# SpeakerGuard/SpeakerGuard

Hardware: AMD Instinct MI355X
Metric: PGD attack steps/sec (xv_plda, 3s@16kHz, batch 64) (higher is better)
Workload: dtype f32; 1 GPU; PGD L-inf eps=0.002 step=0.0004 CE untargeted on xv_plda CSI-E, 64 x 3 s @ 16 kHz per GPU (every rank its own batch), EOT 1/1, dither off; timed = K steps + final forward-only pass; median of 5 attacks; batch_per_gpu=64, samples=48000, global_batch=64

## Files before the change

### speakerguard_amd/csrc/k_conv_gemm.hip

```cpp
#include <atomic>
#include <cstdio>
#include <cstdlib>
#include <vector>
#include <type_traits>

#include "sg_internal.h"

namespace sg {

typedef float f32x16 __attribute__((ext_vector_type(16)));
typedef int i32x4 __attribute__((ext_vector_type(4)));
typedef float f32x4 __attribute__((ext_vector_type(4)));

constexpr int BK = 32;

template <int BM, int BN, int WM, int WN>
__device__ __forceinline__ void gemm_segment(const ConvGemmArgs& p, float* smem, int m0, int n0, int c_begin,
                                             int c_end, f32x16 (&acc)[BM / WM / 32][BN / WN / 32]) {
    constexpr int MI = BM / WM / 32;
    constexpr int NI = BN / WN / 32;
    constexpr int A_QUADS = BM / 4;
    constexpr int B_F4 = BK * BN / 4;
    constexpr int B_PER_THREAD = (B_F4 + 255) / 256;
    static_assert(A_QUADS * 8 <= 256, "A tile too tall");
// ... 708 lines not shown
#pragma unroll
                for (int mi = 0; mi < MI; ++mi) {
                    const float4 x = oa[cur][mi][g];
                    const float xa = st == 0 ? x.x : st == 1 ? x.y : st == 2 ? x.z : x.w;
#pragma unroll
                    for (int ni = 0; ni < NI; ++ni) {
                        const float4 y = BG ? obr[J % DB][ni][h * KGS + g] : ob[cur][ni][g];
                        const float yb = st == 0 ? y.x : st == 1 ? y.y : st == 2 ? y.z : y.w;
                        acc[mi][ni] = __builtin_amdgcn_mfma_f32_32x32x2f32(xa, yb, acc[mi][ni], 0, 0, 0);
                    }
                }
            }
        }
        __builtin_amdgcn_sched_barrier(0);
        __syncthreads();
    };
    const int trips = n / 6;
    for (int q = 0; q < trips; ++q) {
        chunk(std::integral_constant<int, 0>{});
        chunk(std::integral_constant<int, 1>{});
        chunk(std::integral_constant<int, 2>{});
        chunk(std::integral_constant<int, 3>{});
        chunk(std::integral_constant<int, 4>{});
        chunk(std::integral_constant<int, 5>{});
    }
    const int rest = n - 6 * trips;
    if (rest >= 1) chunk(std::integral_constant<int, 0>{});
    if (rest >= 2) chunk(std::integral_constant<int, 1>{});
    if (rest >= 3) chunk(std::integral_constant<int, 2>{});
    if (rest >= 4) chunk(std::integral_constant<int, 3>{});
    if (rest >= 5) chunk(std::integral_constant<int, 4>{});
}

template <int BM, int BN, int WM, int WN, int EPI>
__device__ __forceinline__ void tile_store(const ConvGemmArgs& p, float* C, int m0, int n0,
                                           f32x16 (&acc)[BM / WM / 32][BN / WN / 32]) {
    constexpr int MI = BM / WM / 32;
    constexpr int NI = BN / WN / 32;
    const int lane = threadIdx.x & 63;
    const int wid = __builtin_amdgcn_readfirstlane(threadIdx.x >> 6);
    const int wm = wid / WN, wn = wid % WN;
    const int l31 = lane & 31, lhi = lane >> 5;
    const unsigned lane_off = (unsigned)(4 * lhi * p.ldc + l31) * 4u;
#pragma unroll
    for (int mi = 0; mi < MI; ++mi) {
        const int rowu = m0 + wm * (BM / WM) + mi * 32;
        if (rowu + 32 <= p.M) {
#pragma unroll
            for (int ni = 0; ni < NI; ++ni) {
                const int colu = n0 + wn * (BN / WN) + ni * 32;
                const size_t base = (size_t)rowu * p.ldc + colu;
                float bias = 0.f;
                if (EPI == EPI_BIAS_RELU) bias = p.bias[colu + l31];
                f32x16 mk;
                if (EPI == EPI_RELU_MASK) {
#pragma unroll
                    for (int e = 0; e < 16; ++e) {
                        const char* mb = reinterpret_cast<const char*>(p.mask + base + (size_t)((e & 3) + 8 * (e >> 2)) * p.ldc);
                        mk[e] = *reinterpret_cast<const float*>(mb + lane_off);
                    }
                }
#pragma unroll
                for (int e = 0; e < 16; ++e) {
                    float v = acc[mi][ni][e];
                    if (EPI == EPI_BIAS_RELU) v = fmaxf(v + bias, 0.f);
                    if (EPI == EPI_RELU_MASK) v = mk[e] > 0.f ? v : 0.f;
                    char* cb = reinterpret_cast<char*>(C + base + (size_t)((e & 3) + 8 * (e >> 2)) * p.ldc);
                    *reinterpret_cast<float*>(cb + lane_off) = v;
                }
            }
        } else if (rowu < p.M) {
#pragma unroll
            for (int ni = 0; ni < NI; ++ni) {
                const int col = n0 + wn * (BN / WN) + ni * 32 + l31;
                const int row0 = rowu + 4 * lhi;
                float bias = 0.f;
                if (EPI == EPI_BIAS_RELU) bias = p.bias[col];
                f32x16 mk;
                if (EPI == EPI_RELU_MASK) {
#pragma unroll
                    for (int e = 0; e < 16; ++e) {
                        const int row = min(row0 + (e & 3) + 8 * (e >> 2), p.M - 1);
                        mk[e] = p.mask[(size_t)row * p.ldc + col];
                    }
                }
#pragma unroll
                for (int e = 0; e < 16; ++e) {
                    const int row = row0 + (e & 3) + 8 * (e >> 2);
                    float v = acc[mi][ni][e];
                    if (EPI == EPI_BIAS_RELU) v = fmaxf(v + bias, 0.f);
                    if (EPI == EPI_RELU_MASK) v = mk[e] > 0.f ? v : 0.f;
                    if (row < p.M) C[(size_t)row * p.ldc + col] = v;
                }
            }
        }
    }
}

template <int MI, int NI>
__device__ __forceinline__ void acc_zero(f32x16 (&acc)[MI][NI]) {
#pragma unroll
    for (int mi = 0; mi < MI; ++mi)
#pragma unroll
        for (int ni = 0; ni < NI; ++ni)
#pragma unroll
            for (int e = 0; e < 16; ++e) acc[mi][ni][e] = 0.f;
}

template <int BM, int BN, int WM, int WN, int EPI>
__global__ __launch_bounds__(256, 2) void conv_gemm_kernel(ConvGemmArgs p, int mtiles, int ntiles) {
    __shared__ __attribute__((aligned(16))) float smem[2 * BK * (BM + BN)];
    const int nblk = mtiles * ntiles;
    int bid = blockIdx.x;
    {
        const int q = nblk / 8, r = nblk % 8;
        const int xcd = bid % 8, loc = bid / 8;
        bid = (xcd < r ? xcd * (q + 1) : r * (q + 1) + (xcd - r) * q) + loc;
    }
    const int mt = bid / ntiles, nt = bid % ntiles;
    const int m0 = mt * BM, n0 = nt * BN;
    const int c_begin = blockIdx.z * p.chunks_per_split;
    const int c_end = min(p.total_chunks, c_begin + p.chunks_per_split);
    f32x16 acc[BM / WM / 32][BN / WN / 32];
    acc_zero(acc);
    gemm_segment<BM, BN, WM, WN>(p, smem, m0, n0, c_begin, c_end, acc);
// ... 164 lines not shown
            while (__hip_atomic_load(flags + w - 1, __ATOMIC_RELAXED, __HIP_MEMORY_SCOPE_AGENT) != epoch) {
                __builtin_amdgcn_s_sleep(8);
                if (++spins > ((p.ablate & 8) ? (1u << 12) : (1u << 26))) {
                    if (p.err_word) __hip_atomic_fetch_or(p.err_word, 1u, __ATOMIC_RELAXED, __HIP_MEMORY_SCOPE_SYSTEM);
                    break;
                }
            }
        }
        if (p.ablate & 16) __builtin_amdgcn_fence(__ATOMIC_ACQUIRE, "agent");
        __syncthreads();
        SG_STAMP(9)
        if (computing) {
#pragma unroll
            for (int mi = 0; mi < MI; ++mi)
#pragma unroll
                for (int ni = 0; ni < NI; ++ni)
#pragma unroll
                    for (int q = 0; q < 4; ++q) {
                        const f32x4 v = __builtin_bit_cast(f32x4, __builtin_amdgcn_raw_buffer_load_b128(slab_rsrc, piece_off(w - 1, mi, ni, q), 0, 16));
                        acc[mi][ni][4 * q] = v.x; acc[mi][ni][4 * q + 1] = v.y; acc[mi][ni][4 * q + 2] = v.z; acc[mi][ni][4 * q + 3] = v.w;
                    }
        }
        const int c1 = first_tile == last_tile ? last_c1 : C;
        SG_STAMP(10)
        segment(m0, n0, first_c0, c1, p.trace ? p.trace + (size_t)w * 16 : nullptr);
        SG_STAMP(11)
        if (computing) tile_store<BM, BN, WM, WN, EPI>(p, p.C, m0, n0, acc);
        SG_STAMP(12)
    }
    if (sk_deep(KIND) && p.trace && threadIdx.x == 0) p.trace[(size_t)w * 16 + 14] = __builtin_readcyclecounter();
#undef SG_STAMP
}

template <int BM, int BN, int WM, int WN>
static hipError_t launch_tile(const ConvGemmArgs& a, int epi, int splits, hipStream_t s) {
    const int mtiles = (a.M + BM - 1) / BM;
    const int ntiles = a.N / BN;
    dim3 grid(mtiles * ntiles, 1, splits);
    switch (epi) {
        case EPI_NONE:
            hipLaunchKernelGGL((conv_gemm_kernel<BM, BN, WM, WN, EPI_NONE>), grid, dim3(256), 0, s, a, mtiles, ntiles);
            break;
        case EPI_BIAS_RELU:
            hipLaunchKernelGGL((conv_gemm_kernel<BM, BN, WM, WN, EPI_BIAS_RELU>), grid, dim3(256), 0, s, a, mtiles, ntiles);
            break;
        case EPI_RELU_MASK:
            hipLaunchKernelGGL((conv_gemm_kernel<BM, BN, WM, WN, EPI_RELU_MASK>), grid, dim3(256), 0, s, a, mtiles, ntiles);
            break;
        default:
            return hipErrorInvalidValue;
    }
    return hipGetLastError();
}

typedef float f32x4 __attribute__((ext_vector_type(4)));
template <int EPI, int D, bool TRACE>
__global__ __launch_bounds__(256) void conv_gemm_s16_kernel(ConvGemmArgs p, int ntile32) {
    static_assert(D % 3 == 0, "the LDS stage of a chunk is taken from its ring slot");
    constexpr int A_STAGE = 32 * 32, STAGE = A_STAGE + 8 * 32 * 4;
    __shared__ __attribute__((aligned(16))) float smem[3 * STAGE];
    const int tid = threadIdx.x, lane = tid & 63, wid = tid >> 6;
    const int bm0 = ((int)blockIdx.x / ntile32) * 32, bn0 = ((int)blockIdx.x % ntile32) * 32;
    constexpr unsigned kOob = 0x80000000u;
    const int srow = bm0 + (tid >> 3), c4 = tid & 7;
    const bool srow_ok = srow < p.M;
    const int sb = srow_ok ? srow / p.Tc : 0;
// ... 165 lines not shown
template <int EPI, int KIND>
static void launch_streamk_kind(const ConvGemmArgs& a, int workers, int ntiles, int tiles, int ipw, float* slabs,
                                unsigned* flags, unsigned epoch, hipStream_t s) {
    constexpr int threads = sk_threads(KIND);
    constexpr size_t lds = sk_lds_bytes(KIND);
    static std::atomic<unsigned long long> done_mask{0};
    int dev = 0;
    (void)hipGetDevice(&dev);
    const unsigned long long bit = 1ull << (dev & 63);
    if (!(done_mask.load(std::memory_order_relaxed) & bit)) {
        (void)hipFuncSetAttribute(reinterpret_cast<const void*>(conv_gemm_streamk_kernel<EPI, KIND>),
                                  hipFuncAttributeMaxDynamicSharedMemorySize, (int)lds);
        done_mask.fetch_or(bit, std::memory_order_relaxed);
    }
    hipLaunchKernelGGL((conv_gemm_streamk_kernel<EPI, KIND>), dim3(workers), dim3(threads), lds, s, a, ntiles,
                       tiles, ipw, slabs, flags, epoch);
}

template <int KIND>
static int streamk_blocks_per_cu() {
    static const int n = [] {
        constexpr size_t lds = sk_lds_bytes(KIND);
        const void* fn = reinterpret_cast<const void*>(conv_gemm_streamk_kernel<EPI_NONE, KIND>);
        (void)hipFuncSetAttribute(fn, hipFuncAttributeMaxDynamicSharedMemorySize, (int)lds);
        int nb = 0;
        if (hipOccupancyMaxActiveBlocksPerMultiprocessor(&nb, conv_gemm_streamk_kernel<EPI_NONE, KIND>, sk_threads(KIND), lds) !=
            hipSuccess)
            nb = 0;
        return nb;
    }();
    return n;
}

static hipError_t launch_streamk(const ConvGemmArgs& a, int epi, float* slabs, unsigned* flags, hipStream_t s) {
    static const int w16 = [] {
        const char* e = sg_tune_env("SG_STREAMK_W16");
        return e ? atoi(e) : 1;
    }();
    int kind = !a.Wq ? 0 : ((w16 && a.force != 3) ? 2 : 1);
    const int cus = a.num_cus > 0 && a.num_cus < 256 ? a.num_cus : 256;
    int bm = kind == 2 ? 256 : 128, workers = kind == 2 ? cus : 2 * cus;
    static const int mid = [] {
        const char* e = sg_tune_env("SG_STREAMK_MID");
        return e ? atoi(e) : 1;
    }();
    static const int mid9 = [] {
        const char* e = sg_tune_env("SG_STREAMK_MID9");
        return e ? atoi(e) : 0;
    }();
    if (mid && kind == 2 && a.force == 0 && ((a.M + 255) / 256) * (a.N / 128) < cus) {
        static const int deep = [] {
            const char* e = sg_tune_env("SG_STREAMK_DEEP");
            return e ? atoi(e) : 1;
        }();
        if (((a.M + 127) / 128) * (a.N / 128) >= cus) {
            kind = deep ? (mid9 ? 9 : 5) : 1;
            bm = 128;
            workers = cus;
        } else if (((a.M + 63) / 64) * (a.N / 128) >= cus) {
            kind = deep ? 6 : 3;
            bm = 64;
            workers = cus;
        } else if (((a.M + 31) / 32) * (a.N / 128) >= cus) {
            kind = deep ? 7 : 4;
            bm = 32;
            workers = cus;
        }
// ... 7 lines not shown
        return e ? atoi(e) : 64;
    }();

    if (ws256 && kind == 2 && a.force == 0) {
        if (a.total_chunks >= ws256_min_chunks) {
            kind = 8;
        } else {
            kind = 5;
            bm = 128;
            workers = cus;
        }
    }
    static const int env_kind = [] {
        const char* e = sg_tune_env("SG_STREAMK_KIND");
        return e ? atoi(e) : 0;
    }();
    if (env_kind >= 5 && env_kind <= 9 && a.force == 0 && a.Wq) {
        const int kind0 = kind, bm0 = bm, workers0 = workers;
        kind = env_kind;
        bm = kind == 5 || kind == 9 ? 128 : kind == 6 ? 64 : kind == 7 ? 32 : 256;
        workers = cus;
        const long tl = (long)((a.M + bm - 1) / bm) * (a.N / 128);
        if (tl < workers || (tl * a.total_chunks + workers - 1) / workers < a.total_chunks) {
            kind = kind0;
            bm = bm0;
            workers = workers0;
        }
    }
    if (a.force >= 6 && a.force <= 10 && a.Wq) {
        kind = a.force - 1;
        bm = kind == 5 || kind == 9 ? 128 : kind == 6 ? 64 : kind == 7 ? 32 : 256;
        workers = cus;
    }
    const int mtiles = (a.M + bm - 1) / bm, ntiles = a.N / 128;
    const int tiles = mtiles * ntiles;
    const long total = (long)tiles * a.total_chunks;
    const int ipw = (int)((total + workers - 1) / workers);
    static const int min_chunks = [] {
        const char* e = sg_tune_env("SG_STREAMK_MINCHUNKS");
        return e ? atoi(e) : 16;
    }();
    if (!slabs || !flags || tiles < workers || ipw < a.total_chunks || a.total_chunks < min_chunks) return hipErrorNotSupported;
    const int per_cu = kind == 2 ? streamk_blocks_per_cu<2>() : kind == 1 ? streamk_blocks_per_cu<1>()
                     : kind == 3 ? streamk_blocks_per_cu<3>() : kind == 4 ? streamk_blocks_per_cu<4>()
                     : kind == 5 ? streamk_blocks_per_cu<5>() : kind == 6 ? streamk_blocks_per_cu<6>()
                     : kind == 7 ? streamk_blocks_per_cu<7>() : kind == 8 ? streamk_blocks_per_cu<8>() : kind == 9 ? streamk_blocks_per_cu<9>() : streamk_blocks_per_cu<0>();
    if ((long)per_cu * cus < workers) return hipErrorNotSupported;
    if ((size_t)workers * bm * 128 > (size_t)512 * 128 * 128) return hipErrorNotSupported;
    static std::atomic<unsigned> launch_counter{0};
    unsigned epoch = ++launch_counter;
    if (epoch == 0) epoch = ++launch_counter;
    static const char* trace_file = sg_tune_env("SG_SK_TRACE");
    static const long trace_skip = [] {
        const char* e = sg_tune_env("SG_SK_TRACE_SKIP");
        return e ? atol(e) : 0L;
    }();
    static const long trace_count = [] {
        const char* e = sg_tune_env("SG_SK_TRACE_COUNT");
        return e ? atol(e) : (1L << 60);
    }();
    static std::atomic<long> trace_seen{0};
    static PerDeviceScratch trace_buf;
    bool trace_this = trace_file != nullptr;
    if (trace_this) {
        const long idx = trace_seen.fetch_add(1, std::memory_order_relaxed);
        trace_this = idx >= trace_skip && idx - trace_skip < trace_count;
    }
    unsigned long long* trace_dev = trace_this ? static_cast<unsigned long long*>(trace_buf.get((size_t)workers * 16 * 8)) : nullptr;
    ConvGemmArgs at = a;
    at.trace = trace_dev;
    if (at.lose_counter && *at.lose_counter > 0) {
        at.ablate |= 8;
        --*at.lose_counter;
    }
    at.lose_counter = nullptr;
    dim3 grid(workers);
#define a at
#define SG_SK(EPI)                                                                                          \
    if (kind == 9) launch_streamk_kind<EPI, 9>(a, workers, ntiles, tiles, ipw, slabs, flags, epoch, s);       \
    else if (kind == 8) launch_streamk_kind<EPI, 8>(a, workers, ntiles, tiles, ipw, slabs, flags, epoch, s);  \
    else if (kind == 7) launch_streamk_kind<EPI, 7>(a, workers, ntiles, tiles, ipw, slabs, flags, epoch, s);  \
    else if (kind == 6) launch_streamk_kind<EPI, 6>(a, workers, ntiles, tiles, ipw, slabs, flags, epoch, s);  \
    else if (kind == 5) launch_streamk_kind<EPI, 5>(a, workers, ntiles, tiles, ipw, slabs, flags, epoch, s);  \
    else if (kind == 4) launch_streamk_kind<EPI, 4>(a, workers, ntiles, tiles, ipw, slabs, flags, epoch, s);  \
    else if (kind == 3) launch_streamk_kind<EPI, 3>(a, workers, ntiles, tiles, ipw, slabs, flags, epoch, s);  \
    else if (kind == 2) launch_streamk_kind<EPI, 2>(a, workers, ntiles, tiles, ipw, slabs, flags, epoch, s);  \
    else if (kind == 1) launch_streamk_kind<EPI, 1>(a, workers, ntiles, tiles, ipw, slabs, flags, epoch, s);  \
    else launch_streamk_kind<EPI, 0>(a, workers, ntiles, tiles, ipw, slabs, flags, epoch, s);
    switch (epi) {
        case EPI_NONE: SG_SK(EPI_NONE) break;
        case EPI_BIAS_RELU: SG_SK(EPI_BIAS_RELU) break;
        case EPI_RELU_MASK: SG_SK(EPI_RELU_MASK) break;
        default: return hipErrorInvalidValue;
    }
#undef SG_SK
#undef a
    if (trace_this && trace_dev) {
        std::vector<unsigned long long> h((size_t)workers * 16);
        if (hipStreamSynchronize(s) == hipSuccess &&
            hipMemcpy(h.data(), trace_dev, h.size() * 8, hipMemcpyDeviceToHost) == hipSuccess) {
            if (FILE* f = fopen(trace_file, "ab")) {
                const int hdr[8] = {workers, at.M, at.N, at.total_chunks, ipw, tiles, epi, 0};
                fwrite(hdr, sizeof(hdr), 1, f);
                fwrite(h.data(), 8, h.size(), f);
                fclose(f);
            }
        }
    }
    return hipGetLastError();
}

__global__ void pack_k4_kernel(const float* __restrict__ w, int K, int N, float* __restrict__ wq) {
    const size_t i = (size_t)blockIdx.x * blockDim.x + threadIdx.x;
    if (i >= (size_t)K * N) return;
    const int k = (int)(i / N), n = (int)(i % N);
    wq[((size_t)(k >> 2) * N + n) * 4 + (k & 3)] = w[i];
}

hipError_t launch_pack_k4(const float* w, int K, int N, float* wq, hipStream_t s) {
    const size_t n = (size_t)K * N;
    hipLaunchKernelGGL(pack_k4_kernel, dim3((unsigned)((n + 255) / 256)), dim3(256), 0, s, w, K, N, wq);
    return hipGetLastError();
}

int conv_gemm_tile_rows(int M, int N) {
    (void)M;
    (void)N;
    return 64;
}

hipError_t launch_conv_gemm(const ConvGemmArgs& a_in, int tile, int epi, int splits, hipStream_t s) {
#ifdef SG_EXP_ABLATE
    static const int ablate = [] {
        const char* e = sg_tune_env("SG_ABLATE");
        return e ? atoi(e) : 0;
    }();
#else
    constexpr int ablate = 0;
#endif
    static const int use_streamk = [] {
        const char* e = sg_tune_env("SG_STREAMK");
        return e ? atoi(e) : 1;
    }();
    ConvGemmArgs a = a_in;
    a.ablate |= ablate;
    static const int sk_xcd = [] {
        const char* e = sg_tune_env("SG_STREAMK_XCD");
        return e ? atoi(e) : 2;
    }();
    a.sk_xcd = sk_xcd;
    static const int use_quad = [] {
        const char* e = sg_tune_env("SG_QUADFEED");
        return e ? atoi(e) : 1;
    }();
    if (!use_quad || a.force == 2 || (a.ldw % 4) || (a.Kc % 4)) a.Wq = nullptr;
    if (a.Kc % BK != 0 || a.M <= 0 || a.Tc <= 0) return hipErrorInvalidValue;
    const size_t a_bytes = (size_t)(a.M / a.Tc) * a.Ta * a.lda * sizeof(float);
    const size_t w_bytes = (size_t)a.taps * a.Kc * a.ldw * sizeof(float);
    if (a_bytes >= 0x80000000ull || w_bytes >= 0x80000000ull) return hipErrorInvalidValue;
    a.a_bytes = (unsigned)a_bytes;
    a.w_bytes = (unsigned)w_bytes;
    static const long s16_max = [] {
        const char* e = sg_tune_env("SG_S16_MAX_BLOCKS");
        return e ? atol(e) : 2800L;
    }();
    if ((tile == 0 || tile == 2) && splits == 1 && a.Wq && (a.N % 32) == 0 &&
        (a.force == 5 || (a.force == 0 && a.total_chunks >= 4 && (long)((a.M + 15) / 16) * (a.N / 16) <= s16_max)))
        return launch_s16(a, epi, s);
    switch (tile) {
        case 0: {
            if (a.N % 128) return hipErrorInvalidValue;
            if (splits == 1 && use_streamk && !a.no_streamk && a.force != 1 && a.force != 4) {
                const hipError_t e = launch_streamk(a, epi, a.sk_slabs, a.sk_flags, s);
                if (e != hipErrorNotSupported) return e;
                if (a.force >= 6) return hipErrorInvalidValue;
            }
            if (a.Wq && splits == 1 && a.force != 1) return launch_tile_q(a, epi, s);
            return launch_tile<64, 128, 2, 2>(a, epi, splits, s);
        }
        case 1:
            if (a.N % 32) return hipErrorInvalidValue;
            return launch_tile<128, 32, 4, 1>(a, epi, splits, s);
        case 2:
            if (a.N % 128) return hipErrorInvalidValue;
            if (a.Wq && splits == 1 && a.force != 1) return launch_tile_q(a, epi, s);
            return launch_tile<64, 128, 2, 2>(a, epi, splits, s);
        default:
            return hipErrorInvalidValue;
    }
}

}
```

### speakerguard_amd/csrc/sg_api.hip

```cpp
#include <algorithm>
#include <cmath>
#include <cstdarg>
#include <cstdio>
#include <cstdlib>
#include <cstring>
#include <memory>
#include <type_traits>

#include "sg_internal.h"

using namespace sg;

namespace {

int fail(sg_ctx* ctx, int code, const char* fmt, ...) {
    char buf[512];
    va_list ap;
    va_start(ap, fmt);
    vsnprintf(buf, sizeof(buf), fmt, ap);
    va_end(ap);
    if (ctx) ctx->err = buf;
    return code;
}

// ... 248 lines not shown
    return SG_OK;
}

ConvGemmArgs fwd_layer_args(sg_ctx* ctx, int l, int B, int F) {
    const Workspace& w = ctx->ws;
    ConvGemmArgs a{};
    a.A = l == 0 ? w.feats : w.act[l - 1];
    a.W = ctx->xv.wf[l];
    a.Wq = ctx->xv.wfq[l];
    a.C = w.act[l];
    a.bias = ctx->xv.bias[l];
    a.mask = nullptr;
    a.Ta = l == 0 ? F : w.Fl[l - 1];
    a.Tc = w.Fl[l];
    a.M = B * a.Tc;
    a.N = kCoutPad[l];
    a.Kc = kCinPad[l];
    a.lda = kCinPad[l];
    a.ldw = kCoutPad[l];
    a.ldc = kCoutPad[l];
    a.taps = kTaps[l];
    a.tap_step = kDil[l];
    a.total_chunks = a.taps * (a.Kc / 32);
    a.chunks_per_split = a.total_chunks;
    a.split_stride = 0;
    conv_ctx_args(ctx, a);
    return a;
}

int run_tdnn_forward(sg_ctx* ctx, const PassDims& d, hipStream_t s) {
    Workspace& w = ctx->ws;
    for (int l = 0; l < kLayers; ++l) {
        ConvGemmArgs a = fwd_layer_args(ctx, l, d.B, d.F);
        SG_STAGE(l + 1, launch_conv_gemm(a, 0, EPI_BIAS_RELU, 1, s));
    }
    SG_STAGE(SG_STAGE_POOL_FWD, launch_pool_fwd(w.act[4], d.B, w.Fl[4], w.stats, s));
    ConvGemmArgs a{};
    a.A = w.stats; a.W = ctx->xv.fc1_w; a.C = w.fc1_part; a.bias = nullptr; a.mask = nullptr;
    a.M = d.B; a.N = kEmb; a.Ta = 1; a.Tc = 1; a.Kc = kStats; a.lda = kStats; a.ldw = kEmb; a.ldc = kEmb;
    a.taps = 1; a.tap_step = 0; a.total_chunks = kStats / 32;
    a.chunks_per_split = a.total_chunks / kFc1SplitK;
    a.split_stride = (long long)d.B * kEmb;
    SG_STAGE(SG_STAGE_FC1_FWD, launch_conv_gemm(a, 2, EPI_NONE, kFc1SplitK, s));
    return SG_OK;
}

int run_tdnn_backward(sg_ctx* ctx, const PassDims& d, hipStream_t s) {
    Workspace& w = ctx->ws;
    {
        ConvGemmArgs a{};
        a.A = w.demb; a.W = ctx->xv.fc1_wt; a.C = w.dstats_part; a.bias = nullptr; a.mask = nullptr;
        a.M = d.B; a.N = kStats; a.Ta = 1; a.Tc = 1; a.Kc = kEmb; a.lda = kEmb; a.ldw = kStats; a.ldc = kStats;
        a.taps = 1; a.tap_step = 0; a.total_chunks = kEmb / 32;
        a.chunks_per_split = a.total_chunks / kFc1BwdSplitK;
        a.split_stride = (long long)d.B * kStats;
        SG_STAGE(SG_STAGE_FC1_BWD, launch_conv_gemm(a, 2, EPI_NONE, kFc1BwdSplitK, s));
    }
    SG_STAGE(SG_STAGE_POOL_BWD, launch_pool_bwd(w.act[4], w.stats, w.dstats_part, kFc1BwdSplitK, d.B, w.Fl[4], w.dact[4], s));
    for (int l = kLayers - 1; l >= 0; --l) {
        ConvGemmArgs a{};
        a.A = w.dact[l];
        a.W = ctx->xv.wb[l];
        a.Wq = ctx->xv.wbq[l];
            a.C = l == 0 ? w.dfeats : w.dact[l - 1];
        a.bias = nullptr;
        a.mask = l == 0 ? nullptr : w.act[l - 1];
        a.Ta = w.Fl[l];
        a.Tc = l == 0 ? d.F : w.Fl[l - 1];
        a.M = d.B * a.Tc;
        a.N = kCinPad[l];
        a.Kc = kCoutPad[l];
        a.lda = kCoutPad[l];
        a.ldw = kCinPad[l];
        a.ldc = kCinPad[l];
        a.taps = kTaps[l];
        a.tap_step = -kDil[l];
        a.total_chunks = a.taps * (a.Kc / 32);
        a.chunks_per_split = a.total_chunks;
        a.split_stride = 0;
        conv_ctx_args(ctx, a);
        int splits = 1, tile = 0;
        if (l == 0) {
            tile = 1;
            splits = kL1BwdSplitK;
            a.chunks_per_split = a.total_chunks / kL1BwdSplitK;
            a.split_stride = (long long)d.B * d.F * kFeatPad;
        }
        SG_STAGE(-(l + 1), launch_conv_gemm(a, tile, l == 0 ? EPI_NONE : EPI_RELU_MASK, splits, s));
    }
    return SG_OK;
}

int check_dims(sg_ctx* ctx, int B, int TF, int flag, PassDims* d) {
    if (!ctx) return SG_ERR_ARG;
    if (!ctx->xv.loaded) return fail(ctx, SG_ERR_STATE, "no x-vector model loaded (call sg_xv_load)");
    if (int h = sg_health(ctx)) return h;
    SG_HIP(hipSetDevice(ctx->device));
    if (B < 1) return fail(ctx, SG_ERR_ARG, "B must be >= 1");
    if (flag < 0 || flag > 2) return fail(ctx, SG_ERR_ARG, "flag must be 0 (wav), 1 (raw feat) or 2 (cmvn feat)");
    d->B = B;
    if (flag == SG_FLAG_WAV) {
        if (TF < kWin) return fail(ctx, SG_ERR_ARG, "waveform shorter than one 25 ms window");
        d->T = TF;
        d->F = num_frames(TF);
    } else {
        d->T = 0;
        d->F = TF;
    }
    int Fl[kLayers];
    if (!layer_frames(d->F, Fl)) return fail(ctx, SG_ERR_ARG, "%d frames are too few for the TDNN context", d->F);
    {
        size_t worst = 0;
        for (int l = 0; l < kLayers; ++l) {
// ... 664 lines not shown
```

### speakerguard_amd/csrc/sg_internal.h

```cpp
#pragma once
#include <hip/hip_runtime.h>
#include <cstdlib>
#include <stdint.h>
#include <string>
#include <vector>

#include "../../include/speakerguard_hip.h"

namespace sg {

constexpr int kShift = 160;
constexpr int kWin = 400;
constexpr int kFft = 512;
constexpr int kMel = 30;
constexpr int kCep = 30;
constexpr int kLdaLd = 516;
constexpr int kFeatPad = 32;
constexpr int kCmnWindow = 300;
constexpr float kEps = 1.1920928955078125e-07f;

constexpr int kLayers = 5;
constexpr int kCin[kLayers] = {30, 512, 512, 512, 512};
constexpr int kCout[kLayers] = {512, 512, 512, 512, 1500};
constexpr int kCinPad[kLayers] = {32, 512, 512, 512, 512};
// ... 287 lines not shown
constexpr int kMaxDevices = 64;
inline int sg_device_slot() {
    int d = 0;
    (void)hipGetDevice(&d);
    return d & (kMaxDevices - 1);
}
struct PerDeviceScratch {
    void* ptr[kMaxDevices] = {};
    size_t cap[kMaxDevices] = {};
    void* get(size_t bytes) {
        const int d = sg_device_slot();
        if (cap[d] < bytes) {
            if (ptr[d]) (void)hipFree(ptr[d]);
            ptr[d] = nullptr;
            cap[d] = 0;
            if (hipMalloc(&ptr[d], bytes) == hipSuccess) cap[d] = bytes;
        }
        return ptr[d];
    }
};

inline void conv_ctx_args(sg_ctx* ctx, ConvGemmArgs& a) {
    a.sk_slabs = ctx->sk_slabs;
    a.sk_flags = ctx->sk_flags;
    a.err_word = ctx->err_dev;
    a.num_cus = ctx->num_cus;
    a.no_streamk = ctx->use_streamk ? 0 : 1;
    a.ablate = 0;
    a.lose_counter = ctx->use_streamk ? &ctx->lose_handoffs : nullptr;
}

hipError_t launch_conv_gemm(const ConvGemmArgs& a, int tile, int epi, int splits, hipStream_t s);
int conv_gemm_tile_rows(int M, int N);
hipError_t launch_pack_k4(const float* w, int K, int N, float* wq, hipStream_t s);

hipError_t launch_input_scale(const float* x, int64_t n, float* scratch512, float* scale, int mode, hipStream_t s);
hipError_t launch_mfcc_fwd(const MfccTables& t, const float* x, int B, int T, int F, const float* scale,
                           const sg_dither* dz, float* feats, hipStream_t s);
hipError_t launch_mfcc_bwd(const MfccTables& t, const float* x, int B, int T, int F, const float* scale,
                           const sg_dither* dz, const float* dfeats, float* dframes, hipStream_t s);
hipError_t launch_frames_to_wave(const float* dframes, int B, int T, int F, int R, const float* acc_in, float* grad_out,
                                 float* x_io, const float* lower, const float* upper, float step, int grad_sign,
                                 hipStream_t s);
hipError_t launch_pgd_update(float* x, const float* g, const float* lo, const float* hi, int64_t n,
                             float step, int grad_sign, hipStream_t s);
hipError_t launch_copy_cols(const float* in, int ld_in, float* out, int ld_out, int64_t rows, int ncol, hipStream_t s);
hipError_t launch_sum_cols(const float* in, int ld_in, int nsplit, long long slab_stride, float* out, int ld_out,
                           int64_t rows, int ncol, hipStream_t s);
hipError_t launch_cmvn_fwd(const float* in, int ld_in, float* out, int ld_out, int B, int F, hipStream_t s);
hipError_t launch_cmvn_bwd(const float* dout, int ld_dout, int nsplit, long long slab_stride, float* din, int ld_din,
                           int B, int F, hipStream_t s);
hipError_t launch_pool_fwd(const float* act5, int B, int Tc, float* stats, hipStream_t s);
hipError_t launch_pool_bwd(const float* act5, const float* stats, const float* dstats_part, int nsplit,
                           int B, int Tc, float* dact5, hipStream_t s);

hipError_t launch_cw2_step(float* modifier, float* exp_avg, float* exp_avg_sq, const float* x, const float* input_cur,
                           const float* grad1, const float* const_c, int B, int T, float lr, int step_t,
                           float* input_next, float* loss2, float* scratch, hipStream_t s);
hipError_t launch_nes_queries(const float* x, int n, int T, int half, int with_clean, float sigma, uint64_t seed,
                              int64_t index_base, int pair_base, const float* noise_in, float* queries, float* noise_out,
                              hipStream_t s);
hipError_t launch_nes_grad(const float* loss, int n, int T, int half, int with_clean, uint64_t seed, int64_t index_base,
                           int pair_base, const float* noise_in, int accumulate, float final_sigma, int final_batches,
                           float* grad, hipStream_t s);
hipError_t launch_fakebob_step(float* x, float* grad, const float* prev_grad, const float* lr, const float* lower,
                               const float* upper, int n, int T, float momentum, float one_m_momentum, int grad_sign,
// ... 71 lines not shown
```

Before: 407.2 steps/s.

## Chain two consecutive 1x1 conv GEMMs into one persistent stream-K launch

Adds a chained stream-K kernel that runs two back-to-back 1x1 layer GEMMs (forward layers 4-5 and backward dgrad layers 5-4) inside a single persistent launch. Each worker publishes per-worker completion flags after the first GEMM, and the second GEMM's staging waves spin only on the flags covering the row-tiles they need, so the second layer can start before the whole first layer finishes. The intent is to remove a kernel boundary and its tail/drain idle time. The cost is first-layer stores done as agent-scope atomic writes, extra spin-waits, and more complex host planning that falls back when the chain is not supported.

```diff
diff --git a/speakerguard_amd/csrc/k_conv_gemm.hip b/speakerguard_amd/csrc/k_conv_gemm.hip
--- a/speakerguard_amd/csrc/k_conv_gemm.hip
+++ b/speakerguard_amd/csrc/k_conv_gemm.hip
@@ -764,7 +764,7 @@
     if (rest >= 5) chunk(std::integral_constant<int, 4>{});
 }
 
-template <int BM, int BN, int WM, int WN, int EPI>
+template <int BM, int BN, int WM, int WN, int EPI, bool WT = false>
 __device__ __forceinline__ void tile_store(const ConvGemmArgs& p, float* C, int m0, int n0,
                                            f32x16 (&acc)[BM / WM / 32][BN / WN / 32]) {
     constexpr int MI = BM / WM / 32;
@@ -798,7 +798,8 @@
                     if (EPI == EPI_BIAS_RELU) v = fmaxf(v + bias, 0.f);
                     if (EPI == EPI_RELU_MASK) v = mk[e] > 0.f ? v : 0.f;
                     char* cb = reinterpret_cast<char*>(C + base + (size_t)((e & 3) + 8 * (e >> 2)) * p.ldc);
-                    *reinterpret_cast<float*>(cb + lane_off) = v;
+                    if constexpr (WT) __hip_atomic_store(reinterpret_cast<float*>(cb + lane_off), v, __ATOMIC_RELAXED, __HIP_MEMORY_SCOPE_AGENT);
+                    else *reinterpret_cast<float*>(cb + lane_off) = v;
                 }
             }
         } else if (rowu < p.M) {
@@ -822,7 +823,10 @@
                     float v = acc[mi][ni][e];
                     if (EPI == EPI_BIAS_RELU) v = fmaxf(v + bias, 0.f);
                     if (EPI == EPI_RELU_MASK) v = mk[e] > 0.f ? v : 0.f;
-                    if (row < p.M) C[(size_t)row * p.ldc + col] = v;
+                    if (row < p.M) {
+                        if constexpr (WT) __hip_atomic_store(C + (size_t)row * p.ldc + col, v, __ATOMIC_RELAXED, __HIP_MEMORY_SCOPE_AGENT);
+                        else C[(size_t)row * p.ldc + col] = v;
+                    }
                 }
             }
         }
@@ -1053,6 +1057,153 @@
 #undef SG_STAMP
 }
 
+constexpr int kChainFlagStride = 256;
+template <int EPI, int KIND>
+__global__ __launch_bounds__(sk_threads(KIND), sk_min_waves(KIND)) void conv_gemm_chain_kernel(ConvGemmArgs p1, ConvGemmArgs p2, int mtiles,
+                                                                                    int ntiles1, int ntiles2, int ipw1, int ipw2,
+                                                                                    float* slabs, unsigned* flags, unsigned epoch) {
+    static_assert(KIND >= 5 && KIND <= 7, "the chained launch runs the wave-specialised 128- / 64- / 32-row kinds");
+    constexpr int WM = sk_wm(KIND), WN = sk_wn(KIND);
+    constexpr int BM = sk_bm(KIND), BN = 128;
+    constexpr int MI = BM / WM / 32, NI = BN / WN / 32;
+    constexpr bool BG = sk_bg(KIND);
+    extern __shared__ __attribute__((aligned(16))) float smem[];
+    const int per_xcd = gridDim.x >> 3;
+    const int w = (p1.sk_xcd && (gridDim.x & 7) == 0) ? (blockIdx.x & 7) * per_xcd + (blockIdx.x >> 3) : blockIdx.x;
+    const int lane = threadIdx.x & 63, wid = threadIdx.x >> 6;
+    const bool staging = __builtin_amdgcn_readfirstlane(wid) >= WM * WN;
+    unsigned* const done = flags + 2 * kChainFlagStride;
+    unsigned long long* const tr = p1.trace ? p1.trace + (size_t)w * 16 : nullptr;
+    if (tr && threadIdx.x == 0) {
+        unsigned hw, xcc;
+        asm volatile("s_getreg_b32 %0, hwreg(HW_REG_HW_ID)" : "=s"(hw));
+        asm volatile("s_getreg_b32 %0, hwreg(HW_REG_XCC_ID)" : "=s"(xcc));
+        tr[15] = ((unsigned long long)xcc << 32) | hw;
+        for (int i = 1; i < 15; ++i) tr[i] = 0;
+        tr[0] = __builtin_amdgcn_s_memrealtime();
+    }
+    const unsigned spin_cap = (p1.ablate & 8) ? (1u << 12) : (1u << 26);
+    auto give_up = [&]() {
+        if (p1.err_word) __hip_atomic_fetch_or(p1.err_word, 1u, __ATOMIC_RELAXED, __HIP_MEMORY_SCOPE_SYSTEM);
+    };
+    const int C1 = p1.total_chunks;
+    const long total1 = (long)mtiles * ntiles1 * C1;
+    int ready_mt = -1;
+    auto wait_rows = [&](int mt) {
+        if (mt == ready_mt) return;
+        const long b = (long)mt * ntiles1 * C1, e = min(total1, b + (long)ntiles1 * C1);
+        for (int k = (int)(b / ipw1); k <= (int)((e - 1) / ipw1); ++k) {
+            unsigned spins = 0;
+            while (__builtin_amdgcn_readfirstlane(__hip_atomic_load(done + k, __ATOMIC_RELAXED, __HIP_MEMORY_SCOPE_AGENT)) != epoch) {
+                __builtin_amdgcn_s_sleep(4);
+                if (++spins > spin_cap) {
+                    if (lane == 0) give_up();
+                    break;
+                }
+            }
+        }
+        if (tr && ready_mt < 0 && threadIdx.x == WM * WN * 64) tr[2] = __builtin_amdgcn_s_memrealtime();
+        ready_mt = mt;
+    };
+    f32x16 acc[MI][NI];
+    auto run_layer = [&](const ConvGemmArgs& p, int ntiles, int ipw, int layer) __attribute__((always_inline)) {
+        const int C = p.total_chunks;
+        const long total = (long)mtiles * ntiles * C;
+        const long it_begin = (long)w * ipw;
+        const long it_end = min(total, it_begin + ipw);
+        if (it_begin >= it_end) return;
+        const int first_tile = (int)(it_begin / C), first_c0 = (int)(it_begin % C);
+        const int last_tile = (int)((it_end - 1) / C), last_c1 = (int)((it_end - 1) % C) + 1;
+        const bool head_piece = last_c1 < C, tail_piece = first_c0 > 0;
+        const int whole_begin = tail_piece ? first_tile + 1 : first_tile;
+        const int whole_end = head_piece ? last_tile : last_tile + 1;
+        unsigned* const park = flags + (layer - 1) * kChainFlagStride;
+        const int slab_w = (layer - 1) * (int)gridDim.x + w;
+        auto ready = [&](int tile) {
+            if (layer == 2) wait_rows(tile / ntiles);
+        };
+        if (staging) {
+            if (head_piece && !(last_tile == first_tile && tail_piece)) {
+                ready(last_tile);
+                ws_stage_segment<WM, WN, MI, NI, BG>(p, smem, (last_tile / ntiles) * BM, (last_tile % ntiles) * BN, 0, last_c1);
+                __syncthreads();
+            }
+            for (int tile = whole_begin; tile < whole_end; ++tile) {
+                ready(tile);
+                ws_stage_segment<WM, WN, MI, NI, BG>(p, smem, (tile / ntiles) * BM, (tile % ntiles) * BN, 0, C);
+            }
+            if (tail_piece) {
+                ready(first_tile);
+                __syncthreads();
+                ws_stage_segment<WM, WN, MI, NI, BG>(p, smem, (first_tile / ntiles) * BM, (first_tile % ntiles) * BN, first_c0,
+                                                     first_tile == last_tile ? last_c1 : C);
+            }
+            return;
+        }
+        const __amdgpu_buffer_rsrc_t slab_rsrc = __builtin_amdgcn_make_buffer_rsrc(
+            slabs, 0, (int)min((size_t)2 * gridDim.x * BM * BN * sizeof(float), (size_t)0x7FFFFFFF), 0x00020000);
+        auto piece_off = [&](int wk, int mi, int ni, int q) {
+            return (unsigned)((((size_t)wk * (BM * BN / 4)) + ((((wid * MI + mi) * NI + ni) * 4 + q) * 64 + lane)) * 16);
+        };
+        if (head_piece && !(last_tile == first_tile && tail_piece)) {
+            acc_zero(acc);
+            ws_compute_segment<WM, WN, MI, NI, BG>(p, smem, (last_tile % ntiles) * BN, 0, last_c1, acc);
+#pragma unroll
+            for (int mi = 0; mi < MI; ++mi)
+#pragma unroll
+                for (int ni = 0; ni < NI; ++ni)
+#pragma unroll
+                    for (int q = 0; q < 4; ++q) {
+                        const f32x4 v = {acc[mi][ni][4 * q], acc[mi][ni][4 * q + 1], acc[mi][ni][4 * q + 2], acc[mi][ni][4 * q + 3]};
+                        __builtin_amdgcn_raw_buffer_store_b128(__builtin_bit_cast(i32x4, v), slab_rsrc, piece_off(slab_w, mi, ni, q), 0, 16);
+                    }
+            asm volatile("s_waitcnt vmcnt(0)" ::: "memory");
+            __syncthreads();
+            if (threadIdx.x == 0 && !(p1.ablate & 8)) __hip_atomic_store(park + w, epoch, __ATOMIC_RELAXED, __HIP_MEMORY_SCOPE_AGENT);
+        }
+        for (int tile = whole_begin; tile < whole_end; ++tile) {
+            acc_zero(acc);
+            ws_compute_segment<WM, WN, MI, NI, BG>(p, smem, (tile % ntiles) * BN, 0, C, acc);
+            if (layer == 1) tile_store<BM, BN, WM, WN, EPI, true>(p, p.C, (tile / ntiles) * BM, (tile % ntiles) * BN, acc);
+            else tile_store<BM, BN, WM, WN, EPI>(p, p.C, (tile / ntiles) * BM, (tile % ntiles) * BN, acc);
+        }
+        if (tail_piece) {
+            if (threadIdx.x == 0) {
+                unsigned spins = 0;
+                while (__hip_atomic_load(park + w - 1, __ATOMIC_RELAXED, __HIP_MEMORY_SCOPE_AGENT) != epoch) {
+                    __builtin_amdgcn_s_sleep(8);
+                    if (++spins > spin_cap) {
+                        give_up();
+                        break;
+                    }
+                }
+            }
+            __syncthreads();
+#pragma unroll
+            for (int mi = 0; mi < MI; ++mi)
+#pragma unroll
+                for (int ni = 0; ni < NI; ++ni)
+#pragma unroll
+                    for (int q = 0; q < 4; ++q) {
+                        const f32x4 v = __builtin_bit_cast(f32x4, __builtin_amdgcn_raw_buffer_load_b128(slab_rsrc, piece_off(slab_w - 1, mi, ni, q), 0, 16));
+                        acc[mi][ni][4 * q] = v.x; acc[mi][ni][4 * q + 1] = v.y; acc[mi][ni][4 * q + 2] = v.z; acc[mi][ni][4 * q + 3] = v.w;
+                    }
+            ws_compute_segment<WM, WN, MI, NI, BG>(p, smem, (first_tile % ntiles) * BN, first_c0, first_tile == last_tile ? last_c1 : C, acc);
+            if (layer == 1) tile_store<BM, BN, WM, WN, EPI, true>(p, p.C, (first_tile / ntiles) * BM, (first_tile % ntiles) * BN, acc);
+            else tile_store<BM, BN, WM, WN, EPI>(p, p.C, (first_tile / ntiles) * BM, (first_tile % ntiles) * BN, acc);
+        }
+    };
+    run_layer(p1, ntiles1, ipw1, 1);
+    if (!staging) asm volatile("s_waitcnt vmcnt(0)" ::: "memory");
+    __syncthreads();
+    if (threadIdx.x == 0) {
+        __hip_atomic_store(done + w, epoch, __ATOMIC_RELAXED, __HIP_MEMORY_SCOPE_AGENT);
+        if (tr) tr[1] = __builtin_amdgcn_s_memrealtime();
+    }
+    run_layer(p2, ntiles2, ipw2, 2);
+    if (tr && threadIdx.x == 0) tr[3] = __builtin_amdgcn_s_memrealtime();
+}
+
 template <int BM, int BN, int WM, int WN>
 static hipError_t launch_tile(const ConvGemmArgs& a, int epi, int splits, hipStream_t s) {
     const int mtiles = (a.M + BM - 1) / BM;
@@ -1284,7 +1435,10 @@
     return n;
 }
 
-static hipError_t launch_streamk(const ConvGemmArgs& a, int epi, float* slabs, unsigned* flags, hipStream_t s) {
+struct SkPlan {
+    int kind, bm, workers;
+};
+static SkPlan streamk_plan(const ConvGemmArgs& a) {
     static const int w16 = [] {
         const char* e = sg_tune_env("SG_STREAMK_W16");
         return e ? atoi(e) : 1;
@@ -1358,25 +1512,46 @@
         bm = kind == 5 || kind == 9 ? 128 : kind == 6 ? 64 : kind == 7 ? 32 : 256;
         workers = cus;
     }
-    const int mtiles = (a.M + bm - 1) / bm, ntiles = a.N / 128;
-    const int tiles = mtiles * ntiles;
+    return {kind, bm, workers};
+}
+
+static int streamk_cus(const ConvGemmArgs& a) { return a.num_cus > 0 && a.num_cus < 256 ? a.num_cus : 256; }
+
+static bool streamk_qualifies(const ConvGemmArgs& a, const SkPlan& pl, int& ntiles, int& tiles, int& ipw) {
+    const int mtiles = (a.M + pl.bm - 1) / pl.bm;
+    ntiles = a.N / 128;
+    tiles = mtiles * ntiles;
     const long total = (long)tiles * a.total_chunks;
-    const int ipw = (int)((total + workers - 1) / workers);
+    ipw = (int)((total + pl.workers - 1) / pl.workers);
     static const int min_chunks = [] {
         const char* e = sg_tune_env("SG_STREAMK_MINCHUNKS");
         return e ? atoi(e) : 16;
     }();
-    if (!slabs || !flags || tiles < workers || ipw < a.total_chunks || a.total_chunks < min_chunks) return hipErrorNotSupported;
+    return tiles >= pl.workers && ipw >= a.total_chunks && a.total_chunks >= min_chunks;
+}
+
+static bool streamk_resident(const ConvGemmArgs& a, const SkPlan& pl) {
+    const int kind = pl.kind;
     const int per_cu = kind == 2 ? streamk_blocks_per_cu<2>() : kind == 1 ? streamk_blocks_per_cu<1>()
                      : kind == 3 ? streamk_blocks_per_cu<3>() : kind == 4 ? streamk_blocks_per_cu<4>()
                      : kind == 5 ? streamk_blocks_per_cu<5>() : kind == 6 ? streamk_blocks_per_cu<6>()
                      : kind == 7 ? streamk_blocks_per_cu<7>() : kind == 8 ? streamk_blocks_per_cu<8>() : kind == 9 ? streamk_blocks_per_cu<9>() : streamk_blocks_per_cu<0>();
-    if ((long)per_cu * cus < workers) return hipErrorNotSupported;
-    if ((size_t)workers * bm * 128 > (size_t)512 * 128 * 128) return hipErrorNotSupported;
+    return (long)per_cu * streamk_cus(a) >= pl.workers;
+}
+
+static unsigned streamk_epoch() {
     static std::atomic<unsigned> launch_counter{0};
     unsigned epoch = ++launch_counter;
     if (epoch == 0) epoch = ++launch_counter;
+    return epoch;
+}
+
+static const char* const* streamk_trace_file() {
     static const char* trace_file = sg_tune_env("SG_SK_TRACE");
+    return &trace_file;
+}
+static unsigned long long* streamk_trace_buffer(int workers) {
+    const char* trace_file = *streamk_trace_file();
     static const long trace_skip = [] {
         const char* e = sg_tune_env("SG_SK_TRACE_SKIP");
         return e ? atol(e) : 0L;
@@ -1392,7 +1567,28 @@
         const long idx = trace_seen.fetch_add(1, std::memory_order_relaxed);
         trace_this = idx >= trace_skip && idx - trace_skip < trace_count;
     }
-    unsigned long long* trace_dev = trace_this ? static_cast<unsigned long long*>(trace_buf.get((size_t)workers * 16 * 8)) : nullptr;
+    return trace_this ? static_cast<unsigned long long*>(trace_buf.get((size_t)workers * 16 * 8)) : nullptr;
+}
+static void streamk_trace_write(unsigned long long* trace_dev, int workers, const int (&hdr)[8], hipStream_t s) {
+    std::vector<unsigned long long> h((size_t)workers * 16);
+    if (hipStreamSynchronize(s) == hipSuccess && hipMemcpy(h.data(), trace_dev, h.size() * 8, hipMemcpyDeviceToHost) == hipSuccess) {
+        if (FILE* f = fopen(*streamk_trace_file(), "ab")) {
+            fwrite(hdr, sizeof(hdr), 1, f);
+            fwrite(h.data(), 8, h.size(), f);
+            fclose(f);
+        }
+    }
+}
+
+static hipError_t launch_streamk(const ConvGemmArgs& a, int epi, float* slabs, unsigned* flags, hipStream_t s) {
+    const SkPlan pl = streamk_plan(a);
+    const int kind = pl.kind, bm = pl.bm, workers = pl.workers;
+    int ntiles, tiles, ipw;
+    if (!slabs || !flags || !streamk_qualifies(a, pl, ntiles, tiles, ipw)) return hipErrorNotSupported;
+    if (!streamk_resident(a, pl)) return hipErrorNotSupported;
+    if ((size_t)workers * bm * 128 > (size_t)512 * 128 * 128) return hipErrorNotSupported;
+    const unsigned epoch = streamk_epoch();
+    unsigned long long* trace_dev = streamk_trace_buffer(workers);
     ConvGemmArgs at = a;
     at.trace = trace_dev;
     if (at.lose_counter && *at.lose_counter > 0) {
@@ -1421,17 +1617,77 @@
     }
 #undef SG_SK
 #undef a
-    if (trace_this && trace_dev) {
-        std::vector<unsigned long long> h((size_t)workers * 16);
-        if (hipStreamSynchronize(s) == hipSuccess &&
-            hipMemcpy(h.data(), trace_dev, h.size() * 8, hipMemcpyDeviceToHost) == hipSuccess) {
-            if (FILE* f = fopen(trace_file, "ab")) {
-                const int hdr[8] = {workers, at.M, at.N, at.total_chunks, ipw, tiles, epi, 0};
-                fwrite(hdr, sizeof(hdr), 1, f);
-                fwrite(h.data(), 8, h.size(), f);
-                fclose(f);
-            }
-        }
+    if (trace_dev) {
+        const int hdr[8] = {workers, at.M, at.N, at.total_chunks, ipw, tiles, epi, 0};
+        streamk_trace_write(trace_dev, workers, hdr, s);
+    }
+    return hipGetLastError();
+}
+
+template <int EPI, int KIND>
+static hipError_t launch_chain_kind(const ConvGemmArgs& a1, const ConvGemmArgs& a2, int workers, int mtiles, int nt1, int nt2,
+                                    int ipw1, int ipw2, float* slabs, unsigned* flags, unsigned epoch, hipStream_t s) {
+    constexpr size_t lds = sk_lds_bytes(KIND);
+    static std::atomic<unsigned long long> done_mask{0};
+    int dev = 0;
+    (void)hipGetDevice(&dev);
+    const unsigned long long bit = 1ull << (dev & 63);
+    const void* fn = reinterpret_cast<const void*>(conv_gemm_chain_kernel<EPI, KIND>);
+    if (!(done_mask.load(std::memory_order_relaxed) & bit)) {
+        (void)hipFuncSetAttribute(fn, hipFuncAttributeMaxDynamicSharedMemorySize, (int)lds);
+        done_mask.fetch_or(bit, std::memory_order_relaxed);
+    }
+    int nb = 0;
+    if (hipOccupancyMaxActiveBlocksPerMultiprocessor(&nb, conv_gemm_chain_kernel<EPI, KIND>, sk_threads(KIND), lds) != hipSuccess ||
+        (long)nb * streamk_cus(a1) < workers)
+        return hipErrorNotSupported;
+    hipLaunchKernelGGL((conv_gemm_chain_kernel<EPI, KIND>), dim3(workers), dim3(sk_threads(KIND)), lds, s, a1, a2, mtiles, nt1, nt2,
+                       ipw1, ipw2, slabs, flags, epoch);
+    return hipSuccess;
+}
+
+static hipError_t launch_streamk_chain(const ConvGemmArgs& a1, const ConvGemmArgs& a2, int epi, hipStream_t s) {
+    float* slabs = a1.sk_slabs;
+    unsigned* flags = a1.sk_flags;
+    if (!slabs || !flags || a1.no_streamk || a2.no_streamk || a1.force || a2.force || !a1.Wq || !a2.Wq) return hipErrorNotSupported;
+    if (a1.taps != 1 || a2.taps != 1 || a1.tap_base || a2.tap_base || a2.A != a1.C || a2.M != a1.M || a2.Ta != a1.Tc ||
+        a2.Tc != a1.Tc || a1.Ta != a1.Tc || a2.lda != a1.ldc || a2.Kc != a1.N || a1.sk_xcd == 1 || a2.sk_xcd != a1.sk_xcd)
+        return hipErrorNotSupported;
+    const SkPlan pl = streamk_plan(a1), pl2 = streamk_plan(a2);
+    if (pl.kind < 5 || pl.kind > 7 || pl2.kind != pl.kind || pl2.bm != pl.bm || pl2.workers != pl.workers) return hipErrorNotSupported;
+    int nt1, tiles1, ipw1, nt2, tiles2, ipw2;
+    if (!streamk_qualifies(a1, pl, nt1, tiles1, ipw1) || !streamk_qualifies(a2, pl, nt2, tiles2, ipw2)) return hipErrorNotSupported;
+    const int workers = pl.workers;
+    if (workers > kChainFlagStride || (size_t)2 * workers * pl.bm * 128 > (size_t)512 * 128 * 128) return hipErrorNotSupported;
+    const unsigned epoch = streamk_epoch();
+    unsigned long long* trace_dev = streamk_trace_buffer(workers);
+    ConvGemmArgs b1 = a1, b2 = a2;
+    b1.trace = trace_dev;
+    b2.trace = nullptr;
+    if (b1.lose_counter && *b1.lose_counter > 0) {
+        b1.ablate |= 8;
+        --*b1.lose_counter;
+    }
+    b1.lose_counter = b2.lose_counter = nullptr;
+    const int mtiles = tiles1 / nt1;
+    hipError_t e = hipErrorNotSupported;
+#define SG_CH(EPI)                                                                                                          \
+    if (pl.kind == 5) e = launch_chain_kind<EPI, 5>(b1, b2, workers, mtiles, nt1, nt2, ipw1, ipw2, slabs, flags, epoch, s); \
+    else if (pl.kind == 6) e = launch_chain_kind<EPI, 6>(b1, b2, workers, mtiles, nt1, nt2, ipw1, ipw2, slabs, flags, epoch, s); \
+    else e = launch_chain_kind<EPI, 7>(b1, b2, workers, mtiles, nt1, nt2, ipw1, ipw2, slabs, flags, epoch, s);
+    switch (epi) {
+        case EPI_BIAS_RELU: SG_CH(EPI_BIAS_RELU) break;
+        case EPI_RELU_MASK: SG_CH(EPI_RELU_MASK) break;
+        default: return hipErrorNotSupported;
+    }
+#undef SG_CH
+    if (e != hipSuccess) {
+        if (b1.ablate & 8) ++*a1.lose_counter;
+        return e;
+    }
+    if (trace_dev) {
+        const int hdr[8] = {workers, a1.M, a2.N, a2.total_chunks, ipw2, tiles2, epi, 2};
+        streamk_trace_write(trace_dev, workers, hdr, s);
     }
     return hipGetLastError();
 }
@@ -1455,7 +1711,14 @@
     return 64;
 }
 
-hipError_t launch_conv_gemm(const ConvGemmArgs& a_in, int tile, int epi, int splits, hipStream_t s) {
+static int conv_use_streamk() {
+    static const int use_streamk = [] {
+        const char* e = sg_tune_env("SG_STREAMK");
+        return e ? atoi(e) : 1;
+    }();
+    return use_streamk;
+}
+static hipError_t conv_prepare(ConvGemmArgs& a) {
 #ifdef SG_EXP_ABLATE
     static const int ablate = [] {
         const char* e = sg_tune_env("SG_ABLATE");
@@ -1464,11 +1727,6 @@
 #else
     constexpr int ablate = 0;
 #endif
-    static const int use_streamk = [] {
-        const char* e = sg_tune_env("SG_STREAMK");
-        return e ? atoi(e) : 1;
-    }();
-    ConvGemmArgs a = a_in;
     a.ablate |= ablate;
     static const int sk_xcd = [] {
         const char* e = sg_tune_env("SG_STREAMK_XCD");
@@ -1486,13 +1744,34 @@
     if (a_bytes >= 0x80000000ull || w_bytes >= 0x80000000ull) return hipErrorInvalidValue;
     a.a_bytes = (unsigned)a_bytes;
     a.w_bytes = (unsigned)w_bytes;
+    return hipSuccess;
+}
+static bool conv_takes_s16(const ConvGemmArgs& a, int tile, int splits) {
     static const long s16_max = [] {
         const char* e = sg_tune_env("SG_S16_MAX_BLOCKS");
         return e ? atol(e) : 2800L;
     }();
-    if ((tile == 0 || tile == 2) && splits == 1 && a.Wq && (a.N % 32) == 0 &&
-        (a.force == 5 || (a.force == 0 && a.total_chunks >= 4 && (long)((a.M + 15) / 16) * (a.N / 16) <= s16_max)))
-        return launch_s16(a, epi, s);
+    return (tile == 0 || tile == 2) && splits == 1 && a.Wq && (a.N % 32) == 0 &&
+           (a.force == 5 || (a.force == 0 && a.total_chunks >= 4 && (long)((a.M + 15) / 16) * (a.N / 16) <= s16_max));
+}
+
+hipError_t launch_conv_gemm_chain(const ConvGemmArgs& a1_in, const ConvGemmArgs& a2_in, int epi, hipStream_t s) {
+    static const int use_chain = [] {
+        const char* e = sg_tune_env("SG_CHAIN");
+        return e ? atoi(e) : 1;
+    }();
+    if (!use_chain || !conv_use_streamk()) return hipErrorNotSupported;
+    ConvGemmArgs a1 = a1_in, a2 = a2_in;
+    if (conv_prepare(a1) != hipSuccess || conv_prepare(a2) != hipSuccess) return hipErrorNotSupported;
+    if ((a1.N % 128) || (a2.N % 128) || conv_takes_s16(a1, 0, 1) || conv_takes_s16(a2, 0, 1)) return hipErrorNotSupported;
+    return launch_streamk_chain(a1, a2, epi, s);
+}
+
+hipError_t launch_conv_gemm(const ConvGemmArgs& a_in, int tile, int epi, int splits, hipStream_t s) {
+    const int use_streamk = conv_use_streamk();
+    ConvGemmArgs a = a_in;
+    if (const hipError_t e = conv_prepare(a)) return e;
+    if (conv_takes_s16(a, tile, splits)) return launch_s16(a, epi, s);
     switch (tile) {
         case 0: {
             if (a.N % 128) return hipErrorInvalidValue;
diff --git a/speakerguard_amd/csrc/sg_api.hip b/speakerguard_amd/csrc/sg_api.hip
--- a/speakerguard_amd/csrc/sg_api.hip
+++ b/speakerguard_amd/csrc/sg_api.hip
@@ -304,6 +304,14 @@
     Workspace& w = ctx->ws;
     for (int l = 0; l < kLayers; ++l) {
         ConvGemmArgs a = fwd_layer_args(ctx, l, d.B, d.F);
+        if (l == 3 && !ctx->trace_on) {
+            const hipError_t e = launch_conv_gemm_chain(a, fwd_layer_args(ctx, 4, d.B, d.F), EPI_BIAS_RELU, s);
+            if (e == hipSuccess) {
+                ++l;
+                continue;
+            }
+            if (e != hipErrorNotSupported) SG_HIP(e);
+        }
         SG_STAGE(l + 1, launch_conv_gemm(a, 0, EPI_BIAS_RELU, 1, s));
     }
     SG_STAGE(SG_STAGE_POOL_FWD, launch_pool_fwd(w.act[4], d.B, w.Fl[4], w.stats, s));
@@ -329,7 +337,7 @@
         SG_STAGE(SG_STAGE_FC1_BWD, launch_conv_gemm(a, 2, EPI_NONE, kFc1BwdSplitK, s));
     }
     SG_STAGE(SG_STAGE_POOL_BWD, launch_pool_bwd(w.act[4], w.stats, w.dstats_part, kFc1BwdSplitK, d.B, w.Fl[4], w.dact[4], s));
-    for (int l = kLayers - 1; l >= 0; --l) {
+    auto dgrad_args = [&](int l) {
         ConvGemmArgs a{};
         a.A = w.dact[l];
         a.W = ctx->xv.wb[l];
@@ -351,6 +359,18 @@
         a.chunks_per_split = a.total_chunks;
         a.split_stride = 0;
         conv_ctx_args(ctx, a);
+        return a;
+    };
+    for (int l = kLayers - 1; l >= 0; --l) {
+        ConvGemmArgs a = dgrad_args(l);
+        if (l == 4 && !ctx->trace_on) {
+            const hipError_t e = launch_conv_gemm_chain(a, dgrad_args(3), EPI_RELU_MASK, s);
+            if (e == hipSuccess) {
+                --l;
+                continue;
+            }
+            if (e != hipErrorNotSupported) SG_HIP(e);
+        }
         int splits = 1, tile = 0;
         if (l == 0) {
             tile = 1;
diff --git a/speakerguard_amd/csrc/sg_internal.h b/speakerguard_amd/csrc/sg_internal.h
--- a/speakerguard_amd/csrc/sg_internal.h
+++ b/speakerguard_amd/csrc/sg_internal.h
@@ -343,6 +343,7 @@
 
 hipError_t launch_conv_gemm(const ConvGemmArgs& a, int tile, int epi, int splits, hipStream_t s);
 int conv_gemm_tile_rows(int M, int N);
+hipError_t launch_conv_gemm_chain(const ConvGemmArgs& a1, const ConvGemmArgs& a2, int epi, hipStream_t s);
 hipError_t launch_pack_k4(const float* w, int K, int N, float* wq, hipStream_t s);
 
 hipError_t launch_input_scale(const float* x, int64_t n, float* scratch512, float* scale, int mode, hipStream_t s);
```

Result: no change. 406.8 steps/s (median of 3 runs) (-0.1%).
